# cvxopt/smcp

Measured on AMD Instinct MI355X. Metric: Newton KKT solves/sec, higher is better.
Workload: dtype f64; 1 GPU; synth50k nested block-arrow SDP n=50000, 8073 cliques, m=100; kktsolver=chol, n=50000, cliques=8073, m=100, blkval_doubles=2493568, update_doubles=10689536, parallelism=single

## Files before the change

smcp_amd/csrc/capi.hip:

```cpp
#include <hip/hip_runtime.h>
#include <memory>
#include <unordered_map>

#include <algorithm>
#include <chrono>
#include <cstdio>
#include <cstring>
#include <map>
#include <new>
#include <atomic>
#include <thread>
#include <type_traits>
#include <vector>

#include "../../include/smcp_amd.h"
#include "constraints.hpp"
#include "context.hpp"
#include "hostpar.hpp"
#include "switches.hpp"
#include "front_generic.hip"
#include "front_mfma.hip"
#include "front_large.hip"
#include "front_top.hip"
#include "front_inv.hip"
// ... 529 lines not shown
        if (dyn && tasks > c->D.ncu && tasks < ((int64_t)1 << 30) && c->D.info) {
          static bool attr2 = false;
          if (!attr2) attr2 = hipFuncSetAttribute((const void*)k_lf_assemble_lds_dyn, hipFuncAttributeMaxDynamicSharedMemorySize, 160 * 1024 - 1024) == hipSuccess;
          if (attr2) {
            int* counter = c->D.info + 24 + (st == c->aux_stream[0] ? 1 : (st == c->aux_stream[1] ? 2 : 0));
            (void)hipMemsetAsync(counter, 0, sizeof(int), st);
            launch_lds(c, KID_lf_assemble_lds_dyn, k_lf_assemble_lds_dyn, dim3(c->D.ncu), dim3(1024), bytes, st, a, U, ldu, sgn, cnt, nrhs, nz, counter);
            return;
          }
        }
        launch_lds(c, KID_lf_assemble_lds, k_lf_assemble_lds, dim3(cnt, nrhs, nz), dim3(1024), bytes, st, a, U, ldu, sgn);
        return;
      }
    }
  }
  if (a.chskip) launch(c, KID_lf_clear_upd, k_lf_zero_skipped, dim3(cnt, nrhs), dim3(256), st, a);
  if (clear_first && !(plan && a.t.gp_tptr && c->plan_full_upd))
    launch(c, KID_lf_clear_upd, k_lf_clear_upd, dim3(umax1(std::min(64, (a.namax * a.namax + 2047) / 2048)), cnt, nrhs), dim3(256), st, a);
  if (plan && a.t.gp_tptr) {
    const int nfm = a.nnmax + a.namax;
    const int gx = (int64_t)cnt * nrhs * 32 < 2 * (int64_t)c->D.ncu ? std::max(32, std::min(128, (nfm * (nfm + 1) / 2 + 255) / 256)) : 32;
    if (a.nchmax <= 8) launch(c, KID_lf_assemble, k_lf_assemble<8>, dim3(gx, cnt, nrhs), dim3(256), st, a, U, ldu, sgn);
    else launch(c, KID_lf_assemble, k_lf_assemble<16>, dim3(gx, cnt, nrhs), dim3(256), st, a, U, ldu, sgn);
    return;
  }
  const int nfmax = a.nnmax + a.namax;
  const int ncb = (nfmax + LF_TW - 1) / LF_TW, nrb = (nfmax + LF_TR - 1) / LF_TR;
  launch(c, KID_lf_assemble, k_lf_assemble_tiled, dim3(ncb * nrb, cnt, nrhs), dim3(256), st, a, U, ldu, sgn);
}

static bool pd_deep() {
  static int on = -1;
  if (on < 0) { const char* e = sw_str("SMCP_PD"); on = (e && e[0] == '1') ? 0 : 1; }
  return on == 1;
}
static int64_t pd_wgs() {
  static int64_t v = -1;
  if (v < 0) { const char* e = sw_str("SMCP_PD_WGS"); v = e ? std::max(1, atoi(e)) : 1; }
  return v;
}
#define LAUNCH_PD(c, kid, kern, grid, blk, ...)                                                        \
  do {                                                                                                 \
    const dim3 g_ = (grid);                                                                            \
    if (pd_deep() && (int64_t)g_.x * g_.y * g_.z <= pd_wgs() * (int64_t)(c)->D.ncu) launch(c, kid, kern<4>, g_, dim3(1024), __VA_ARGS__); \
    else launch(c, kid, kern<1>, g_, blk, __VA_ARGS__);                                                \
  } while (0)

constexpr int ROOT_FUSED_MAXNN = 512;
static bool root_fused() {
  static int on = -1;
  if (on < 0) { const char* e = sw_str("SMCP_ROOT_FUSED"); on = (e && e[0] == '1') ? 1 : 0; }
  return on == 1;
}
void lf_up(csp_ctx* c, const MfmaArgs& a, int cnt, int nrhs, double* U, int64_t ldu, hipStream_t st, bool fill = false) {
  const int mtA = tiles64(a.namax), ntN = tiles64(a.nnmax);
  dim3 blk(256);
  if (a.nchmax > 0) {
    lf_assemble(c, a, cnt, nrhs, U, ldu, fill ? 3 : 0, st, true);
    if (c->mid_work && a.level >= 2) {
      std::function<void(hipStream_t)> w = std::move(c->mid_work);
      c->mid_work = nullptr;
      w(st);
    }
    if (c->side_work) {
      std::function<void(hipStream_t)> w = std::move(c->side_work);
      c->side_work = nullptr;
      Fork* f = new Fork(c, st, 1);
      c->side_fork = f;
      w(f->s);
    }
  }
  LAUNCH_PD(c, KID_lf_up1, k_lf_up1, dim3(umax1(mtA * ntN + ntN * ntN), cnt, nrhs), blk, st, a, U, ldu);
  LAUNCH_PD(c, KID_lf_up2, k_lf_up2, dim3(umax1(mtA * (mtA + 1) / 2 + mtA * ntN + ntN * (ntN + 1) / 2), cnt, nrhs), blk, st, a, U, ldu);
  if (a.namax) LAUNCH_PD(c, KID_lf_up3, k_lf_up3, dim3(umax1(mtA * ntN), cnt, nrhs), blk, st, a, U, ldu);
}
void lf_down(csp_ctx* c, const MfmaArgs& a, int cnt, int nrhs, double* U, int64_t ldu, hipStream_t st) {
  const int mtA = tiles64(a.namax), ntN = tiles64(a.nnmax);
  dim3 blk(256);
  if (a.namax) launch(c, KID_gather_level, k_gather_level, dim3(cnt, nrhs, gather_parts(a.namax, (int64_t)cnt * nrhs, c->D.ncu)), dim3(NT), st, a.t, (const double*)U, ldu, a.t.upd);
  LAUNCH_PD(c, KID_lf_down1, k_lf_down1, dim3(umax1(mtA * ntN + ntN * ntN), cnt, nrhs), blk, st, a, U, ldu);
  if (a.namax) LAUNCH_PD(c, KID_lf_down2, k_lf_down2, dim3(umax1(mtA * ntN), cnt, nrhs), blk, st, a, U, ldu);
  LAUNCH_PD(c, KID_lf_down3, k_lf_down3, dim3(umax1(ntN * (ntN + 1) / 2), cnt, nrhs), blk, st, a, U, ldu);
}
void lf_pinv(csp_ctx* c, const MfmaArgs& a, int cnt, double* x, hipStream_t st) {
  const int mtA = tiles64(a.namax), ntN = tiles64(a.nnmax);
  dim3 blk(256);
  if (a.namax) {
    launch(c, KID_gather_level, k_gather_level, dim3(cnt, 1, gather_parts(a.namax, cnt, c->D.ncu)), dim3(NT), st, a.t, (const double*)x, (int64_t)0, a.t.upd);
    LAUNCH_PD(c, KID_lf_pinv1, k_lf_pinv1, dim3(umax1(mtA * ntN), cnt, 1), blk, st, a, x);
  }
  LAUNCH_PD(c, KID_lf_pinv2, k_lf_pinv2, dim3(umax1(ntN * (ntN + 1) / 2 + mtA * ntN), cnt, 1), blk, st, a, x);
}

constexpr size_t LF_DIAG_LDS = (size_t)(2 * LB * LBD + 256 + 16 * LB) * sizeof(double);
static dim3 diag_blk() {
  static int t = 0;
  if (!t) { const char* e = sw_str("SMCP_DIAG_THREADS"); t = e ? atoi(e) : 512; if (t < 64 || t > 1024 || (t & 63)) t = 512; }
  return dim3(t);
}

bool use_mid(int rowsmax) {
  static int g = -1;
  if (g < 0) {
    const char* e = sw_str("SMCP_MID");
    g = (e && e[0] == '0') ? 0 : 1;
    if (g && hipFuncSetAttribute((const void*)k_mid_chol, hipFuncAttributeMaxDynamicSharedMemorySize, (int)mid_chol_lds(MID_MAXROWS)) != hipSuccess) g = 0;
  }
  return g == 1 && rowsmax <= MID_MAXROWS;
}
bool flow_chol(csp_ctx* c, hipStream_t st, double* A, int64_t ld, int n, double* dinv, const MfmaArgs* fa, int mode, int* info, int info_val, int cnt = 1) {
  static int on = -1, wgs = 0;
  if (on < 0) { on = sw_on("SMCP_FLOW", 1); wgs = std::max(1, std::min(FLOW_MAXWG, sw_int("SMCP_FLOW_WG", FLOW_MAXWG))); }
  if (!on || use_generic(c) || n <= 2 * LB || n > FLOW_MAXN || !info) return false;
  if (cnt < 1 || (cnt > 1 && (!fa || dinv || cnt > wgs / 8))) return false;
  static int attr = -1;
  if (attr < 0) attr = hipFuncSetAttribute((const void*)k_chol_flow, hipFuncAttributeMaxDynamicSharedMemorySize, (int)FLOW_LDS_BYTES) == hipSuccess ? 1 : 0;
  if (!attr) return false;
  const int nt = (n + 63) / 64, ntiles = nt * (nt + 1) / 2;
  csp_ctx::FlowWs& W = c->flow_ws[st == c->aux_stream[0] && st ? 1 : (st == c->aux_stream[1] && st ? 2 : 0)];
  if (W.cap_nt < nt || W.cap_fronts < cnt) {
    const int ntc = std::max(nt, W.cap_nt), ntilesc = ntc * (ntc + 1) / 2, frc = std::max(cnt, W.cap_fronts);
    DevLedger& mem = c->D.mem;
    W.epoch = 0;
    if (dev_grow(&W.P, &W.len_P, (int64_t)frc * ntilesc * 4096, mem, st) || dev_grow(&W.dinv, &W.len_dinv, (int64_t)frc * ntc * 4096, mem, st) ||
        dev_grow(&W.flags, &W.len_flags, (int64_t)frc * (ntilesc + ntc + 4), mem, st) ||
        hipMemset(W.flags, 0, sizeof(unsigned) * (size_t)W.len_flags) != hipSuccess) {
      (void)hipGetLastError();
      (void)dev_free(mem, W.P, W.dinv, W.flags);
      W = csp_ctx::FlowWs();
      return false;
    }
    W.cap_nt = ntc; W.cap_fronts = frc;
  }
  const int wgs_front = cnt > 1 ? wgs / cnt : (n > 2048 ? (wgs * 10) / 7 : wgs);
  if ((int64_t)ntiles > (int64_t)FLOW_MAXOWN * wgs_front) return false;
  const int plan_key = n * 1024 + std::min(1023, wgs_front);
  auto it = c->flow_plans.find(plan_key);
  if (it == c->flow_plans.end()) {
    std::vector<int32_t> optr, otile;
    flow_make_plan(n, wgs_front, optr, otile);
    csp_ctx::FlowPlanDev P;
    P.nwg = (int)optr.size() - 1;
    if (dev_upload(&P.own_ptr, optr, c->D.mem) || dev_upload(&P.own_tile, otile, c->D.mem)) {
      (void)hipGetLastError();
      (void)dev_free(c->D.mem, P.own_ptr, P.own_tile);
      return false;
    }
    it = c->flow_plans.emplace(plan_key, P).first;
  }
  FlowArgs f;
  f.A = A; f.ld = ld; f.n = n;
  f.dinv = dinv ? dinv : W.dinv;
  f.P = W.P; f.flags = W.flags;
  f.epoch = ++W.epoch;
  f.own_ptr = it->second.own_ptr; f.own_tile = it->second.own_tile;
  f.info = info; f.info_val = info_val;
  f.cl = fa ? fa->t.cl : nullptr; f.lev = fa ? fa->t.lev : nullptr; f.mode = mode; f.nsn1 = fa ? fa->t.nsn1 : 1;
  f.dbg = nullptr;
  f.p_stride = (int64_t)ntiles * 4096; f.dinv_stride = (int64_t)nt * 4096; f.flag_stride = ntiles + nt + 4;
  static int stamps = -1;
  if (stamps < 0) stamps = sw_on("SMCP_FLOW_STAMPS", 0);
  static long long* dbg = nullptr;
  if (stamps) { if (!dbg) (void)hipMalloc((void**)&dbg, sizeof(long long) * 16 * FLOW_MAXWG); f.dbg = dbg; }
  launch_lds(c, KID_chol_flow, k_chol_flow, dim3(it->second.nwg, cnt), dim3(256), FLOW_LDS_BYTES, st, f);
  if (stamps && dbg) {
    std::vector<long long> h((size_t)8 * it->second.nwg);
    (void)hipStreamSynchronize(st);
    (void)hipMemcpy(h.data(), dbg, h.size() * sizeof(long long), hipMemcpyDeviceToHost);
    for (int w = 0; w < std::min(it->second.nwg, 20); ++w)
      fprintf(stderr, "flow n %d wg %3d: idle %7.1f us (%lld)  update %7.1f us (%lld)  potrf %7.1f us (%lld)  panel %7.1f us (%lld)\n", n, w,
              h[8 * w] / 100.0, h[8 * w + 4], h[8 * w + 1] / 100.0, h[8 * w + 5], h[8 * w + 2] / 100.0, h[8 * w + 6], h[8 * w + 3] / 100.0, h[8 * w + 7]);
// ... 1152 lines not shown
    case CSP_Q_EDM_CLAMPED:
      if (out) out[0] = c->edm_clamped;
      return 1;
    case CSP_Q_CEIG_SWEEPS:
      if (out) out[0] = c->ceig_sweeps;
      return 1;
  }
  return SMCP_EINVAL;
}

int csp_maxcardsearch(int64_t n, const int64_t* colptr, const int64_t* rowind, int64_t* order) {
  if (n <= 0 || !colptr || !rowind || !order) return SMCP_EINVAL;
  maxcardsearch(n, colptr, rowind, order);
  return 0;
}
int csp_mindegree(int64_t n, const int64_t* colptr, const int64_t* rowind, int64_t* order) {
  if (n <= 0 || !colptr || !rowind || !order) return SMCP_EINVAL;
  mindegree(n, colptr, rowind, order);
  return 0;
}
int csp_index_map(const csp_ctx* c, int64_t cnt, const int64_t* I, const int64_t* J, int64_t* out) {
  if (!c || cnt < 0) return SMCP_EINVAL;
  index_map(c->S, cnt, I, J, out);
  return 0;
}

}

#include "setup.hip"

namespace {

struct ScalFam {
  bool on = false;
  MfmaArgs af;
  int nfam = 0;
  const int32_t* lone = nullptr;
  int nlone = 0, lnn = 0, lna = 0;
  int nfmax = 0, cpan = 0, sel = 0;
  size_t bytes = 0;
};
ScalFam scaling_fam_plan(csp_ctx* c, const MfmaArgs& a0, int set) {
  ScalFam p;
  static const int on = sw_on("SMCP_SCALING_FAM", 1);
  if (!on || set || use_generic(c) || fam_off() || c->verify_cache || c->ntrial != 1 || c->sets[1].lev2 || c->sets[2].lev2 || c->S.nlev < 2) return p;
  const LevelClass& L0 = c->lvl[0];
  const LevelClass& L1 = c->lvl[1];
  if (!L1.nI || !L1.nS || !L0.nS) return p;
  for (int64_t l = 2; l < c->S.nlev; ++l) if (c->lvl[(size_t)l].nS) return p;
  if (L1.famnn > 16 || L1.famna > 64 || L1.famcnn > 16 || L1.famcna > 32) return p;
  p.af = a0;
  p.af.t.lev = c->D.lev2idx + c->S.levptr[1] + (L1.nI - L1.nS);
  p.af.level = 1;
  p.af.famna = L1.famna; p.af.famnn = L1.famnn; p.af.famcna = L1.famcna; p.af.famcnn = L1.famcnn;
  p.nfam = (int)L1.nS;
  const int nout = (int)(L0.nI - L0.nS);
  if (nout > 0 && L0.nnmaxI <= 16 && L0.namaxI <= 64) { p.lone = c->D.lev2idx + c->S.levptr[0]; p.nlone = nout; p.lnn = L0.nnmaxI; p.lna = L0.namaxI; }
  p.nfmax = std::max(L1.famnn + L1.famna, p.lnn + p.lna);
  p.cpan = (L1.famcnn + L1.famcna) * L1.famcnn;
  p.bytes = sfam_lds_bytes(p.nfmax, p.cpan);
  if (p.bytes > 64 * 1024) return p;
  const int pnat = (std::max(std::max((int)L1.famna, p.lna), 1) + 15) / 16, cnat = (std::max((int)L1.famcna, 1) + 15) / 16;
  p.sel = 2 * pnat + cnat;
  p.on = p.sel >= 3 && p.sel <= 10;
  return p;
}
template <bool PREP>
bool launch_chol_fam(csp_ctx* c, const ScalFam& p, double* x, double* lkout, hipStream_t st) {
  const dim3 grid(p.nfam + p.nlone), blk(256);
#define SMCP_CF(PN, CN) launch_lds(c, KID_chol_fam, k_chol_fam<PN, CN, PREP>, grid, blk, p.bytes, st, p.af, x, lkout, p.nfmax, p.cpan, p.nfam, p.lone); return true
  switch (p.sel) {
    case 3: SMCP_CF(1, 1);
    case 4: SMCP_CF(1, 2);
    case 5: SMCP_CF(2, 1);
    case 6: SMCP_CF(2, 2);
    case 7: SMCP_CF(3, 1);
    case 8: SMCP_CF(3, 2);
    case 9: SMCP_CF(4, 1);
    case 10: SMCP_CF(4, 2);
  }
#undef SMCP_CF
  return false;
}
bool launch_pinv_fam(csp_ctx* c, const ScalFam& p, const MfmaArgs& ap, double* x, hipStream_t st) {
  MfmaArgs af = p.af;
  af.t.upd = ap.t.upd; af.LK = ap.LK;
  const dim3 grid(p.nfam + p.nlone), blk(256);
#define SMCP_PF(PN, CN) launch_lds(c, KID_pinv_fam, k_pinv_fam<PN, CN>, grid, blk, p.bytes, st, af, x, p.nfmax, p.cpan, p.nfam, p.lone); return true
  switch (p.sel) {
    case 3: SMCP_PF(1, 1);
    case 4: SMCP_PF(1, 2);
    case 5: SMCP_PF(2, 1);
    case 6: SMCP_PF(2, 2);
    case 7: SMCP_PF(3, 1);
    case 8: SMCP_PF(3, 2);
    case 9: SMCP_PF(4, 1);
    case 10: SMCP_PF(4, 2);
  }
#undef SMCP_PF
  return false;
}
template <class Small, class Large, class Fam>
void scaling_fam_up(csp_ctx* c, const ScalFam& p, const MfmaArgs& a0, Small small, Large large, Fam fam) {
  for (int64_t l = 0; l < 2; ++l) {
    if (l == 1) fam();
    for_level_classes(c, l, a0, [&](bool lds, MfmaArgs am, int cnt, size_t, int thr) {
      if (!lds) { large(am, cnt, l); return; }
      cnt -= am.nS;
      if (cnt > 0 && !(l == 0 && p.nlone)) small(am, cnt, thr);
    });
  }
}
template <class Small, class Large, class Fam>
void scaling_fam_down(csp_ctx* c, const ScalFam& p, const MfmaArgs& a0, Small small, Large large, Fam fam) {
  for (int64_t l = 1; l >= 0; --l) {
    if (l == 0) fam();
    for_level_classes(c, l, a0, [&](bool lds, MfmaArgs am, int cnt, size_t, int thr) {
      if (!lds) { large(am, cnt, l); return; }
      cnt -= am.nS;
      if (cnt > 0 && !(l == 0 && p.nlone)) small(am, cnt, thr);
    });
  }
}

}

extern "C" {

int64_t csp_device_bytes(const csp_ctx* c) { return c ? c->D.mem.total : 0; }

static int cholesky_impl(csp_ctx* c, double* x, void* stream, int set, bool li_last = false);
int csp_cholesky(csp_ctx* c, double* x, void* stream) { return cholesky_impl(c, x, stream, 0); }
int csp_cholesky_part(csp_ctx* c, double* x, int set, void* stream) {
  if (set < 1 || set > 2 || !c || !c->sets[set].lev2 || use_generic(c)) return SMCP_EINVAL;
  return cholesky_impl(c, x, stream, set);
}
static int cholesky_impl(csp_ctx* c, double* x, void* stream, int set, bool li_last) {
  if (int rc = ready(c)) return rc;
  invalidate_tags(c, x);
  hipStream_t st = (hipStream_t)stream;
  TreeArgs a = tree_args(c);
  HIPCHK(zero_flag(c, st));
  if (!use_generic(c)) {
    MfmaArgs a0 = mfma_args(c, nullptr, 0, 1);
    a0.LK = nullptr;
    auto small = [&](const MfmaArgs& am, int cnt, int thr) {
      launch_lds(c, KID_chol_mfma, k_chol_mfma<true>, dim3(cnt), dim3(fact_threads(am, thr, 0)),
                 (size_t)mfma_lds_doubles_for(WK_CHOL, am.nnmax, am.namax) * sizeof(double), st, am, x, (double*)nullptr);
    };
    auto large = [&](const MfmaArgs& am, int cnt, int64_t l) {
      if (use_large() && c->D.gp_tptr) lf_chol(c, am, cnt, x, st, li_last && l == c->S.nlev - 1);
      else launch_lds(c, KID_chol_mfma_hbm, k_chol_mfma<false>, dim3(cnt), dim3(1024), 0, st, am, x, (double*)nullptr);
    };
    const ScalFam sf = scaling_fam_plan(c, a0, set);
    if (sf.on) scaling_fam_up(c, sf, a0, small, large, [&]() { launch_chol_fam<false>(c, sf, x, (double*)nullptr, st); });
    for (int64_t l = sf.on ? 2 : 0; l < c->S.nlev; ++l)
      for_level_classes(c, l, a0, [&](bool lds, MfmaArgs am, int cnt, size_t bytes, int thr) {
        (void)bytes;
        if (lds) small(am, cnt, thr);
        else large(am, cnt, l);
      }, set);
  } else
  for_levels_up(c, [&](const int32_t* lev, int cnt) {
    a.lev = lev;
    launch(c, KID_chol_level, k_chol_level, dim3(cnt), dim3(NT), st, a, x);
  });
  HIPCHK(end_call(c));
  return fetch_info(c, st);
}

int csp_llt(csp_ctx* c, double* x, void* stream) {
// ... 94 lines not shown
  if (c->scal_lstar < 0) {
    int64_t ls = S.nlev;
    while (ls > 0 && c->lvl[(size_t)ls - 1].nI == 0) --ls;
    c->scal_lstar = ls;
    std::vector<int> lev_of((size_t)S.nsn, 0);
    for (int64_t l = 0; l < S.nlev; ++l)
      for (int64_t q = S.levptr[l]; q < S.levptr[l + 1]; ++q) lev_of[(size_t)S.levidx[q]] = (int)l;
    int64_t t0 = bl;
    for (int64_t k = 0; k < S.nsn; ++k) if (lev_of[(size_t)k] == S.nlev - 1) t0 = std::min<int64_t>(t0, S.blkptr[k]);
    for (int64_t k = 0; k < S.nsn; ++k) if (S.blkptr[k] >= t0 && lev_of[(size_t)k] != S.nlev - 1) { t0 = 0; break; }
    c->scal_tail0 = t0;
  }
  const int64_t lstar = c->scal_lstar;
  const bool fast = !use_generic(c) && use_large() && D.gp_tptr && !cache_off() && Fork::enabled() && scaling_overlap_on() &&
                    c->ntrial == 1 && lstar < S.nlev && (lstar > 0 || D.nI_total == 0) && D.yaa && S.updlen() > 0 && !c->verify_cache;
  if (!fast) {
    const bool li = top_li_whole(c);
    if (li) { D.lk_tag_L = D.lk_tag_Y = nullptr; D.part_valid = false; D.lk_gen++; }
    if (int rc = cholesky_impl(c, L, (void*)st, 0, li)) return rc;
    HIPCHK(hipMemcpyAsync(Y, L, sizeof(double) * bl, hipMemcpyDeviceToDevice, st));
    if (int rc = projected_inverse_impl(c, Y, (void*)st, 0, li)) return rc;
    c->D.lk_tag_L = L;
    if (flags & SCALING_FAC) { if (int rc = prepare_yaa(c, Y, true, st)) return rc; HIPCHK(end_call(c)); }
    return 0;
  }
  invalidate_tags(c, L);
  invalidate_tags(c, Y);
  HIPCHK(zero_flag(c, st));
  const int64_t last = S.nlev - 1;
  const int64_t tail0 = c->scal_tail0;
  MfmaArgs a0 = mfma_args(c, nullptr, 0, 1);
  a0.LK = nullptr;
  TreeArgs t = tree_args(c);
  int nnI = 0;
  for (const LevelClass& Lc : c->lvl) if (Lc.nI) nnI = std::max(nnI, (int)Lc.nnmaxI);
  static int cprep = -1;
  if (cprep < 0) { const char* e = sw_str("SMCP_CHOL_PREP"); cprep = (e && e[0] == '0') ? 0 : 1; }
  const bool fuse_prep = cprep && nnI <= 16;
  auto chol_small = [&](const MfmaArgs& am, int cnt, int thr) {
    const size_t lb = (size_t)mfma_lds_doubles_for(WK_CHOL, am.nnmax, am.namax) * sizeof(double);
    if (fuse_prep) launch_lds(c, KID_chol_mfma, k_chol_mfma<true, true>, dim3(cnt), dim3(fact_threads(am, thr, 0)), lb, st, am, L, D.lk);
    else launch_lds(c, KID_chol_mfma, k_chol_mfma<true>, dim3(cnt), dim3(fact_threads(am, thr, 0)), lb, st, am, L, (double*)nullptr);
  };
  auto chol_large = [&](const MfmaArgs& am, int cnt, int64_t l) { lf_chol(c, am, cnt, L, st, l == last); };
  auto chol_level = [&](int64_t l) {
    for_level_classes(c, l, a0, [&](bool lds, MfmaArgs am, int cnt, size_t bytes, int thr) {
      (void)bytes;
      if (lds) chol_small(am, cnt, thr);
      else chol_large(am, cnt, l);
    });
  };
  const ScalFam sf = scaling_fam_plan(c, a0, 0);
  if (sf.on)
    scaling_fam_up(c, sf, a0, chol_small, chol_large, [&]() {
      if (fuse_prep) launch_chol_fam<true>(c, sf, L, D.lk, st);
      else launch_chol_fam<false>(c, sf, L, (double*)nullptr, st);
    });
  for (int64_t l = sf.on ? 2 : 0; l < last; ++l) chol_level(l);
  std::unique_ptr<Fork> f0;
  if (last > 0) f0.reset(new Fork(c, st, 1));
  hipStream_t s0 = f0 ? f0->s : st;
  chol_level(last);
  if (D.nI_total && !fuse_prep) {
    TreeArgs ts = t;
    ts.lev = D.lev3idx;
    launch_lds(c, KID_prep_lk, k_prep_lk, dim3((int)D.nI_total), dim3(prep_lk_threads(nnI)), prep_lk_lds_bytes(nnI), s0, ts, (const double*)L, D.lk);
  }
  for (int64_t ll = 0; ll < last; ++ll)
    for_level_classes(c, ll, a0, [&](bool lds, MfmaArgs am, int cnt, size_t, int) { if (!lds) lf_prep(c, am, cnt, L, s0); });
  if (tail0 > 0) (void)hipMemcpyAsync(Y, L, sizeof(double) * tail0, hipMemcpyDeviceToDevice, s0);
  for_level_classes(c, last, a0, [&](bool lds, MfmaArgs am, int cnt, size_t, int) { if (!lds) lf_prep(c, am, cnt, L, st, use_top(am.nnmax + am.namax)); });
  (void)hipMemcpyAsync(Y + tail0, L + tail0, sizeof(double) * (bl - tail0), hipMemcpyDeviceToDevice, st);
  if (f0) f0->join();
  D.lk_gen++;
  D.part_valid = false;
  MfmaArgs ap = mfma_args(c, nullptr, 0, 1);
  ap.t.upd = D.yaa;
  MfmaArgs af = mfma_args(c, nullptr, 0, 1);
  const bool want_fac = (flags & SCALING_FAC) != 0;
  static int skipenv = -1;
  if (skipenv < 0) { const char* e = sw_str("SMCP_FAC_PARTIAL"); skipenv = (e && e[0] == '0') ? 0 : 1; }
  const bool skip_children = want_fac && skipenv && D.m > 0 && !D.ns && leafgram_ok(c, D.m) && c->leafgram_policy != 0;
  bool skipped = false;
  auto factor_level = [&](int64_t l, hipStream_t lds_stream, hipStream_t large_stream) {
    for_level_classes(c, l, af, [&](bool lds, MfmaArgs am, int cnt, size_t, int) {
      if (!am.namax) return;
      if (lds) {
        if (l == 0 && skip_children && am.nS > 0) { cnt -= am.nS; skipped = true; if (!cnt) return; }
        const size_t bytes = ((size_t)padld(am.namax) * am.namax + 256 + 8) * sizeof(double);
        launch_lds(c, KID_factor_yaa_lds, k_factor_yaa_lds, dim3(cnt), dim3(fact_threads(am, 256, 2)), bytes, lds_stream, am, (const double*)D.yaa, D.fac);
      } else {
        launch(c, KID_axpby, k_copy_upd_blocks, dim3(cnt, umax1(std::min(64, (am.namax * am.namax + 1023) / 1024))), dim3(256), large_stream,
               am.t, (const double*)D.yaa, D.fac);
        lf_factor_yaa(c, am, cnt, D.fac, large_stream);
      }
    });
  };
  auto pinv_small = [&](const MfmaArgs& am, int cnt, int thr) {
    launch_lds(c, KID_pinv_mfma, k_pinv_mfma<true>, dim3(cnt), dim3(fact_threads(am, thr, 1)),
               (size_t)mfma_lds_doubles_for(WK_PINV, am.nnmax, am.namax) * sizeof(double), st, am, Y);
  };
  auto pinv_large = [&](const MfmaArgs& am, int cnt, int64_t) { lf_pinv(c, am, cnt, Y, st); };
  auto pinv_level = [&](int64_t l) {
    for_level_classes(c, l, ap, [&](bool lds, MfmaArgs am, int cnt, size_t bytes, int thr) {
      (void)bytes;
      if (lds) pinv_small(am, cnt, thr);
      else pinv_large(am, cnt, l);
    });
  };
  for (int64_t l = last; l >= lstar; --l) pinv_level(l);
  bool any_large_sep = false;
  for (int64_t l = lstar; l <= last; ++l) if (c->lvl[(size_t)l].nII && c->lvl[(size_t)l].namaxII > 0) any_large_sep = true;
  std::unique_ptr<Fork> f1;
  if (want_fac && any_large_sep && lstar > 0) f1.reset(new Fork(c, st, 0));
  hipStream_t s1 = f1 ? f1->s : st;
  for (int64_t l = lstar - 1; l >= (sf.on ? 2 : 0); --l) pinv_level(l);
  if (sf.on) scaling_fam_down(c, sf, ap, pinv_small, pinv_large, [&]() { launch_pinv_fam(c, sf, ap, Y, st); });
  if (want_fac) {
    for (int64_t l = last; l >= lstar; --l) factor_level(l, s1, s1);
    for (int64_t l = lstar - 1; l >= 0; --l) factor_level(l, st, st);
  }
  if (f1) f1->join();
  D.lk_tag_L = L; D.lk_tag_Y = Y;
  D.yaa_tag = Y;
  D.fac_tag = want_fac ? Y : nullptr;
  D.fac_partial = want_fac && skipped;
  D.faci_tag = nullptr;
  if (want_fac) D.fac_gen++;
  HIPCHK(end_call(c));
  const int rc = fetch_info(c, st);
  if (rc) {
    D.lk_tag_L = D.lk_tag_Y = D.yaa_tag = D.fac_tag = D.faci_tag = nullptr;
    D.part_valid = false;
  }
  return rc;
}
int csp_cholesky_projected_inverse(csp_ctx* c, double* L, double* Y, int with_factors, void* stream) {
  if (int rc = ready(c)) return rc;
  if (!L || !Y || L == Y) return SMCP_EINVAL;
  return scaling_impl(c, L, Y, with_factors ? SCALING_FAC : 0, (hipStream_t)stream);
}

int csp_completion(csp_ctx* c, double* x, void* stream) {
  if (int rc = ready(c)) return rc;
  invalidate_tags(c, x);
  hipStream_t st = (hipStream_t)stream;
  TreeArgs a = tree_args(c);
  HIPCHK(zero_flag(c, st));
  if (!use_generic(c)) {
    prepare_yaa(c, x, true, st, true);
    MfmaArgs a0 = mfma_args(c, c->D.faci, 0, 1);
    a0.LK = nullptr;
    dim3 blk(256);
    for (int64_t l = 0; l < c->S.nlev; ++l)
      for_level_classes(c, l, a0, [&](bool lds, MfmaArgs am, int cnt, size_t bytes, int thr) {
        const size_t cb = lds ? (size_t)completion_lds_doubles(am.nnmax, am.namax) * sizeof(double) : 0;
        if (lds && cb <= LDS_LIMIT) {
          launch_lds(c, KID_completion_mfma, k_completion_mfma<true>, dim3(cnt), dim3(cb > 48 * 1024 ? 512 : 256), cb, st, am, x);
        }
        else if (lds || !use_large())
          launch_lds(c, KID_completion_mfma_hbm, k_completion_mfma<false>, dim3(cnt), dim3(lds ? 256 : thr), 0, st, am, x);
      });
    if (use_large())
      for_all_large(c, a0, [&](MfmaArgs am, int cnt) {
        const int mtA = tiles64(am.namax), ntN = tiles64(am.nnmax);
        if (am.namax) {
          launch(c, KID_lf_completion, k_lf_completion, dim3(umax1(mtA * ntN), cnt), blk, st, am, x, 0);
          launch(c, KID_lf_completion, k_lf_completion, dim3(umax1(mtA * ntN), cnt), blk, st, am, x, 1);
        }
        launch(c, KID_lf_completion, k_lf_completion, dim3(umax1(ntN * ntN), cnt), blk, st, am, x, 2);
        if (use_mid(am.nnmax))
          launch_lds(c, KID_mid_chol, k_mid_chol, dim3(cnt), dim3(1024), mid_chol_lds(am.nnmax), st, am, (double*)nullptr, (double*)nullptr, 3);
        else
        for (int jb = 0; jb < am.nnmax; jb += LB) {
          launch_lds(c, KID_lf_diag, k_lf_diag, dim3(cnt), diag_blk(), LF_DIAG_LDS, st, am, (double*)nullptr, (double*)nullptr, 3, jb, 1);
          const int mrem = am.nnmax - jb - 1;
          if (mrem > 0) {
            launch(c, KID_lf_chol_panel, k_lf_chol_panel, dim3(umax1(tiles64(mrem)), cnt), blk, st, am, (double*)nullptr, (double*)nullptr, 3, jb);
            const int mt = tiles64(mrem);
            launch(c, KID_lf_chol_trail, k_lf_chol_trail, dim3(umax1(mt * (mt + 1) / 2), cnt), blk, st, am, (double*)nullptr, (double*)nullptr, 3, jb);
          }
        }
        for (int ib = 0; ib < am.nnmax; ib += LB) {
          launch_lds(c, KID_lf_diag, k_lf_diag, dim3(cnt), diag_blk(), LF_DIAG_LDS, st, am, (double*)nullptr, (double*)nullptr, 3, ib, 0);
          if (ib > 0) launch(c, KID_lf_prep_s, k_lf_prep_s, dim3(umax1(tiles64(ib)), cnt), blk, st, am, (const double*)nullptr, (double*)nullptr, ib, 3);
          launch(c, KID_lf_prep_row, k_lf_prep_row, dim3(umax1(tiles64(ib) + 1), cnt), blk, st, am, (const double*)nullptr, (double*)nullptr, ib, 3, 0);
        }
        launch(c, KID_lf_completion, k_lf_completion, dim3(umax1(ntN * ntN + mtA * ntN), cnt), blk, st, am, x, 3);
      });
    invalidate_tags(c, x);
  } else {
    gather_all(c, x, 0, 1, c->D.upd, st);
    launch(c, KID_completion_all, k_completion_all, dim3((int)c->S.nsn), dim3(NT), st, a, x);
  }
  HIPCHK(end_call(c));
  return fetch_info(c, st);
}

int csp_hessian(csp_ctx* c, const double* L, const double* Y, double* U, int64_t nrhs, int64_t ldu,
                int adj, int inv, void* stream) {
  if (int rc = ready(c)) return rc;
  if (nrhs < 1 || adj < 0 || adj > 2 || (nrhs > 1 && ldu < c->S.blklen())) return SMCP_EINVAL;
// ... 286 lines not shown
```

smcp_amd/csrc/front_pinvfam.hip:

```cpp
#include <hip/hip_runtime.h>

namespace smcp {

template <int NAT, bool OWN, int M>
__device__ inline d4 pinv_fam_tiles(const double (&li)[4], const double (&kk)[4 * M], const CliqueDesc& d, double* P, double* yaa,
                                    double* zs, int nfz, const int32_t* rel, int t0, int t1, bool with_li, int lane) {
  const int l15 = lane & 15, kq = lane >> 4;
  const int nn = d.nn, na = d.na, nf = nn + na;
  const int ksn = (nn + 3) >> 2, ksa = (na + 3) >> 2;
  const d4 zero4 = {0.0, 0.0, 0.0, 0.0};
  d4 accN = zero4;
  if (with_li) {
#pragma unroll
    for (int s = 0; s < 4; ++s)
      if (s < ksn) fmma(accN, li[s], li[s]);
  }
#pragma unroll
  for (int t = 0; t < NAT; ++t) {
    if (t < t0 || t >= t1 || 16 * t >= na) continue;
    const int m = 16 * t + l15;
    int ri = 0;
    if (!OWN) ri = rel[min(m, na - 1)];
    d4 accE = zero4;
#pragma unroll
    for (int s0 = 0; s0 < 4 * NAT; s0 += 8) {
      double y[8];
#pragma unroll
      for (int s = s0; s < s0 + 8 && s < 4 * NAT; ++s) {
        const int j = kq + 4 * s;
        const int i1 = OWN ? nn + min(m, na - 1) : ri, j1 = OWN ? nn + min(j, na - 1) : rel[min(j, na - 1)];
        const double v = zs[pk_low(max(i1, j1), min(i1, j1), nfz)];
        y[s - s0] = (m < na && j < na) ? v : 0.0;
        if (!OWN && m < na && j <= m) yaa[m + j * na] = v;
      }
#pragma unroll
      for (int s = s0; s < s0 + 8 && s < 4 * NAT; ++s)
        if (s < ksa) fmma(accE, kk[s], y[s - s0]);
    }
#pragma unroll
    for (int rr = 0; rr < 4; ++rr) {
      const int mm = 16 * t + kq + 4 * rr;
      if (mm < na && l15 < nn) {
        P[nn + mm + l15 * nf] = -accE[rr];
        if (OWN) zs[pk_low(nn + mm, l15, nfz)] = -accE[rr];
      }
    }
#pragma unroll
    for (int s = 0; s < 4; ++s) fmma(accN, kk[4 * t + s], accE[s]);
  }
  return accN;
}

template <int PNAT, int CNAT>
__global__ void __launch_bounds__(256, 4) k_pinv_fam(MfmaArgs a, double* x, int nfmax, int cpan, int nfam, const int32_t* lone) {
  extern __shared__ double zs[];
  const int tid = threadIdx.x;
  const int lane = tid & 63, l15 = lane & 15, kq = lane >> 4;
  const int wave = __builtin_amdgcn_readfirstlane((int)(threadIdx.x >> 6));
  const int k = (int)blockIdx.x < nfam ? a.t.lev[blockIdx.x] : lone[(int)blockIdx.x - nfam];
  const CliqueDesc d = a.t.cl[k];
  const int nn = d.nn, na = d.na, nf = nn + na;
  const int nch = (int)blockIdx.x < nfam ? d.chend - d.chbeg : 0;
  double* const P = x + d.blk;
  const bool has0 = wave < nch, has1 = wave + 4 < nch;
  const CliqueDesc dc0 = a.t.cl[has0 ? a.t.chidx[d.chbeg + wave] : k];
  const CliqueDesc dc1 = a.t.cl[has1 ? a.t.chidx[d.chbeg + wave + 4] : k];
  const SfamStage st = sfam_stage_of(zs, nfmax, wave, cpan);
  if (has0) { sfam_stage(st, a.LK + dc0.blk, (dc0.nn + dc0.na) * dc0.nn, lane); sfam_stage_rel(st, a.t, dc0, lane); }
  constexpr int M = PNAT > CNAT ? PNAT : CNAT;
  double li[4], kk[4 * M];
  down_fam_load_lk<PNAT, M>(li, kk, a.LK + d.blk, d, lane);
  if (na > 0) {
    const bool haspar = d.parent >= 0;
    const CliqueDesc par = a.t.cl[haspar ? d.parent : k];
    const int nng = par.nn, nag = par.na, nfg = nng + nag;
    const double* Pg = x + par.blk;
    const double* Ug = a.t.upd + par.upd;
    double* const UkG = a.t.upd + d.upd;
    const int32_t* rel = a.t.relidx + d.rel;
    const int gi = rel[min(lane, na - 1)];
    double v[4 * PNAT];
#pragma unroll
    for (int c = 0; c < 4 * PNAT; ++c) {
      const int j = wave + 4 * c;
      v[c] = 0.0;
      if (haspar && j < na && lane >= j && lane < na) {
        const int gj = rel[j];
        const int hi = max(gi, gj), lo = min(gi, gj);
        v[c] = lo < nng ? Pg[hi + (int64_t)lo * nfg] : Ug[(hi - nng) + (int64_t)(lo - nng) * nag];
      }
    }
#pragma unroll
    for (int c = 0; c < 4 * PNAT; ++c) {
      const int j = wave + 4 * c;
      if (j < na && lane >= j && lane < na) {
        zs[pk_low(nn + lane, nn + j, nf)] = v[c];
        if (haspar) UkG[lane + j * na] = v[c];
      }
    }
  }
  __syncthreads();
  {
    const d4 accN = pinv_fam_tiles<PNAT, true, M>(li, kk, d, P, nullptr, zs, nf, nullptr, wave, wave + 1, wave == 0, lane);
#pragma unroll
    for (int rr = 0; rr < 4; ++rr) st.D[l15 + 16 * (kq + 4 * rr)] = accN[rr];
  }
  __syncthreads();
  {
    const int i = tid & 15, j = tid >> 4;
    if (i < nn && j <= i) {
      double v = sfam_stage_of(zs, nfmax, 0, cpan).D[tid];
#pragma unroll
      for (int w = 1; w < 4; ++w)
        if (w < PNAT && 16 * w < na) v += sfam_stage_of(zs, nfmax, w, cpan).D[tid];
      zs[pk_low(i, j, nf)] = v;
      P[i + j * nf] = v;
    }
  }
  if (nch == 0) return;
  __syncthreads();
  const int pan1 = (dc1.nn + dc1.na) * dc1.nn;
  const bool pre1 = has1 && pan1 <= 256;
  SfamPre pre;
  if (has0) {
    down_fam_load_lk<CNAT, M>(li, kk, st.P, dc0, lane);
    if (pre1) sfam_fetch(pre, a.LK + dc1.blk, pan1, a.t, dc1, lane);
  }
  auto child = [&](const CliqueDesc& dc) {
    double* const Pc = x + dc.blk;
    const d4 accN = pinv_fam_tiles<CNAT, false, M>(li, kk, dc, Pc, a.t.upd + dc.upd, zs, nf, st.rel, 0, CNAT, true, lane);
    const int nfc = dc.nn + dc.na;
#pragma unroll
    for (int rr = 0; rr < 4; ++rr) {
      const int c = kq + 4 * rr;
      if (l15 < dc.nn && c <= l15) Pc[l15 + c * nfc] = accN[rr];
    }
  };
  if (has0) child(dc0);
  if (has1) {
    wave_sync();
    if (pre1) sfam_commit(st, pre, pan1, dc1, lane);
    else { sfam_stage(st, a.LK + dc1.blk, pan1, lane); sfam_stage_rel(st, a.t, dc1, lane); }
    wave_sync();
    down_fam_load_lk<CNAT, M>(li, kk, st.P, dc1, lane);
    child(dc1);
  }
}

}
```

smcp_amd/csrc/switches.hpp:

```cpp
#pragma once
#include <cstdio>
#include <cstdlib>
#include <cstring>
#include <string>

extern char** environ;

namespace smcp {

struct Switch { const char* name; const char* dflt; const char* doc; };

static const Switch SWITCHES[] = {
  {"SMCP_GENERIC", "0", "1: any-size fixed-order kernels of front_generic.hip for every tree operation (as CSP_TUNE_DETERMINISTIC)"},
  {"SMCP_LARGE", "1", "0: no tiled large-front kernels (fronts beyond LDS take the one-workgroup HBM kernels)"},
  {"SMCP_NOCACHE", "0", "1: nothing derived from (L, Y) is reused between calls"},
  {"SMCP_FORK", "1", "0: no side streams, everything on the caller's stream"},
  {"SMCP_AUX_PRIO", "1", "0: side stream 0 (few-workgroup chains) at default instead of highest priority"},
  {"SMCP_AUX_PRIO1", "1", "0: side stream 1 (filler work) at default instead of lowest priority"},
  {"SMCP_EVENT_SYSFENCE", "0", "1: internal events with the default system-scope release (12 us per hand-over instead of 7)"},
  {"SMCP_SCALING_OVERLAP", "1", "0: csp_cholesky_projected_inverse as its three steps one after the other"},
  {"SMCP_CHOL_PREP", "1", "0: k_prep_lk in a launch of its own instead of inside k_chol_mfma (narrow supernodes)"},
  {"SMCP_FAC_PARTIAL", "1", "0: chol(Y_AA) of the family children always formed by the fused scaling point"},
  {"SMCP_MID", "1", "0: per-step kernels instead of k_mid_chol / k_lf_diag_inv for fronts of at most 272 rows"},
  {"SMCP_TOP_FUSED", "1", "0: k_mid_chol, and k_lf_diag_inv / k_lf_trtri for the inverse at the scaling point, instead of the register-resident k_top_chol for fronts of at most 208 rows"},
  {"SMCP_TRTRI", "1", "0: block-row triangular inversion of large fronts instead of recursive doubling"},
  {"SMCP_N16", "1", "0: no shape-specialised k_hess_up_n16"},
  {"SMCP_OLDLDS", "0", "1: k_hess_up_mfma<true> instead of the padded / n16 kernels"},
  {"SMCP_DOWN_W", "1", "0: k_hess_down_mfma instead of the one-wave k_hess_down_w"},
  {"SMCP_DOWN_FAM", "1", "most right-hand sides of a root -> leaves sweep that take the one-launch family kernel k_hess_down_fam (0: never; the per-level k_hess_down_w launches)"},
  {"SMCP_UP_FAM", "1", "most dense right-hand sides of a leaves -> root sweep that take the resident family kernel k_hess_up_fam1, the level-0 cliques outside the families riding along (0: never; k_hess_up_fam and a launch of their own for those cliques)"},
  {"SMCP_SCALING_FAM", "1", "0: per-level k_chol_mfma / k_pinv_mfma launches for the families of the scaling point instead of one k_chol_fam / k_pinv_fam launch each way"},
  {"SMCP_FAM", "1", "0: no family kernels (per-level sweeps with the update exchange through HBM)"},
  {"SMCP_FAM2", "1", "0: no sparse-input family kernels (k_fam_sparse, k_fam_terms): k_hess_up_fam"},
  {"SMCP_FAMT", "1", "0: no entry-driven family sweep k_fam_terms (k_fam_sparse instead)"},
  {"SMCP_FZ", "1", "0: the family parents' packed updates go through HBM (k_fam_terms writes, the extend-add reads) instead of being formed by k_lf_assemble_fz"},
  {"SMCP_FAMT_GROUP", "1", "0: no sibling groups of family parents (k_fam_terms_grp)"},
  {"SMCP_LFSP", "1", "0: dense phases instead of the sparse-input sweep k_lfsp_up of childless large fronts"},
  {"SMCP_LFSP_GROUP", "1", "0: no sibling groups in k_lfsp_up"},
  {"SMCP_ZSP", "1", "0: dense first phase of wide childless fronts instead of k_lf_zsp"},
  {"SMCP_LEAFGRAM", "1", "0: never the closed-form Gram blocks of the family children (k_leaf_tables / k_leaf_pairs)"},
  {"SMCP_LG_SIDE", "1", "0: leaf Gram blocks after the sweep on the caller's stream instead of beside the top phases"},
  {"SMCP_GRAM_EARLY", "0", "1: the Gram chunks of the levels 0 / 1 rows on the side branch beside the top fronts' phase kernels (measured slower: 3.37 against 3.22 ms per step)"},
  {"SMCP_LG_EARLY", "1", "0: leaf Gram blocks beside the phase kernels of the top fronts instead of from the start of the sweep"},
  {"SMCP_FACI_LDS", "1", "0: inverse Y_AA factors of the small fronts by block rows against HBM (k_factor_inverse) instead of in LDS"},
  {"SMCP_FZ_TAIL", "1", "0: every (front, right-hand side) pair of the fused extend-add is one workgroup's task, also in a thin last round"},
  {"SMCP_GRAM", "1", "0: reference (two-sweep) formulation of the Schur complement instead of the Gram formulation"},
  {"SMCP_SCM", "1", "0: column-sparse constraints swept like the others (no SCMcolumn2 route)"},
  {"SMCP_TRSM_MM", "1", "0: csp_trsm through the generic level kernels instead of tile products"},
  {"SMCP_TRMM_MM", "1", "0: no MFMA tile products in csp_trmm (every front on the FMA kernels); 2: tile products for the large fronts only, also from 32 columns on"},
  {"SMCP_SYR2K_MM", "1", "0: no MFMA tile products in csp_syr2k (every front on the FMA kernel); 2: tile products for the large fronts only, whatever the rank (read on every call)"},
  {"SMCP_SYMM_MM", "1", "0: no MFMA tile products in csp_symm (every front on the FMA kernel); 2: tile products for the large fronts only, whatever the column count (read on every call)"},
  {"SMCP_LOWRANK_MM", "1", "0: no MFMA tiles in the Gram products of the low-rank factor (k_lr_gram on the FMA route whatever the shape)"},
  {"SMCP_POTRS_MANY_MM", "1", "0: no MFMA tile products in the block steps of dense_potrs_many / kkt_solve_many (FMA updates whatever the column count; read on every call)"},
  {"SMCP_ALDS", "1", "0: extend-add of large fronts by gather plan only (no LDS streaming kernel)"},
  {"SMCP_ALDS_DYN", "1", "0: one workgroup per (front, right-hand side) instead of the task-drawing grid"},
  {"SMCP_ALDS_FILL", "1", "0: k_panel_fill builds the input panels instead of the extend-add (sgn 3)"},
  {"SMCP_ASM", "plan", "t: tiled extend-add kernel instead of the gather plan"},
  {"SMCP_ROOT_FUSED", "0", "1: fused two-product sweep of fronts without separator (Y_NN explicit: condition squared; studies only)"},
  {"SMCP_PD", "0", "1: four-wave tile products everywhere (no sixteen-wave shape for small launches)"},
  {"SMCP_FLOW", "1", "0: no one-launch blocked Cholesky with in-launch tile dataflow (front_flow.hip): per-step kernels for dense matrices / single fronts beyond 272 rows"},
  {"SMCP_FLOW_WG", "112", "workgroups of that launch (at most 112: four launches fit the chip side by side)"},
  {"SMCP_POTRF_DEFER", "1", "0: kkt_schur_factor factors H at once even under deferred status"},
  {"SMCP_QR_TRSM", "mfma", "f: vector-FMA substitution kernel of kkt_qr instead of the MFMA one"},
  {"SMCP_FTHR_CHOL", "128", "threads of k_chol_mfma on the leaf class"},
  {"SMCP_FTHR_PINV", "256", "threads of k_pinv_mfma on the leaf class"},
  {"SMCP_FTHR_YAA", "64", "threads of k_factor_yaa_lds on the leaf class"},
  {"SMCP_FTHR_YAA_MID", "256", "threads of k_factor_yaa_lds on separator blocks of 33 .. 64 rows"},
  {"SMCP_N16_THR_LEAF", "128", "threads of k_hess_up_n16 for one or two right-hand sides on childless fronts"},
  {"SMCP_DIAG_THREADS", "512", "threads of k_lf_diag"},
  {"SMCP_POTRF_THREADS", "1024", "threads of k_dense_potrf_small"},
  {"SMCP_FZ_THREADS", "1024", "threads of k_lf_assemble_fz (512: eight waves, no register spills, slower)"},
  {"SMCP_PD_WGS", "1", "largest launch, in workgroups per CU, that takes the sixteen-wave tile shape"},
  {"SMCP_ALDS_Z", "0", "workgroups per (front, right-hand side) of the LDS extend-add (0: automatic)"},
  {"SMCP_RHS_SPLIT", "16", "fewest right-hand sides for the two-stream split of a large-front sweep (plain extend-add launch only)"},
  {"SMCP_RHS_PARTS", "2", "parts of that split (2 or 3)"},
  {"SMCP_RHS_SPLIT_DYN", "0", "1: the split also with the task-drawing extend-add"},
  {"SMCP_FAM_MINRHS", "1", "fewest dense right-hand sides for the family kernel"},
  {"SMCP_FAMT_G", "0", "right-hand-side slices per family of k_fam_terms (0: cost model)"},
  {"SMCP_FAM2_STAG", "0", "stagger of k_fam_sparse's groups (studies)"},
  {"SMCP_FAMT_MEAN", "36", "entry-driven family sweeps (k_fam_terms, fused extend-add) up to this many entries per (family, constraint) list ON AVERAGE (lists up to 384 entries, in chunks); beyond: the dense family sweep"},
  {"SMCP_LFSP_OCC", "2", "waves per SIMD the grouped update phase of k_lfsp_up is compiled for (1: 512 registers, no spills; 2: 256, ~100 spilled)"},
  {"SMCP_LFSP_G", "1", "right-hand sides per workgroup of k_lfsp_up"},
  {"SMCP_GRAM_NW", "16", "waves per workgroup of k_gram_diag128 (4, 8 or 16)"},
  {"SMCP_GRAM_MINCHUNK", "512", "fewest stack rows per workgroup of the Gram accumulation"},
  {"SMCP_UPDP_PAD", "0", "doubles of padding between the packed exchange buffers of consecutive right-hand sides"},
  {"SMCP_QR_PASSES", "0", "Cholesky-QR passes of kkt_qr (0: decided by the deviation test)"},
  {"SMCP_QR_P", "1", "positions per lane of the FMA substitution kernel (1 or 2)"},
  {"SMCP_FLOW_STAMPS", "0", "1: per-workgroup time accounts of the one-launch blocked Cholesky on stderr (waits for every launch)"},
  {"SMCP_POISON", "0", "1: every fp64 device buffer of the library (and the exchange buffers of smcp_amd/kkt.py) starts as 4.5e150 (hunting reads of never-written workspace)"},
  {"SMCP_RACE", "0", "seed > 0: delay injection on every internal stream hand-over and one launch in eight (race hunting; results must not change)"},
  {"SMCP_TRACE", "0", "1: every launch named on stderr and waited for (a device fault points at its kernel)"},
  {"SMCP_TIMING", "0", "1: wall-clock marks of the set-up phases on stderr"},
  {"SMCP_OCC", "0", "1: occupancy decisions of k_hess_up_n16 on stderr"},
  {"SMCP_DEBUG_ADDR", "0", "1: addresses of the large allocations on stderr"},
  {"SMCP_CONTIG", "0", "1: large buffers from physically contiguous memory (placement studies: slower)"},
  {"SMCP_SKIP", "0", "phase mask of the sweep kernels (ablation timing; results are wrong)"},
  {"SMCP_GSKIP", "0", "ablation mask of the Gram kernel (results are wrong)"},
  {"SMCP_LGSKIP", "0", "ablation mask of k_leaf_pairs (results are wrong)"},
  {"SMCP_QR_FAKE", "0", "1: timing experiment of the FMA substitution kernel (results are wrong)"},
};

inline void sw_check_environment() {
  static const bool done = [] {
    for (char** e = environ; e && *e; ++e) {
      if (std::strncmp(*e, "SMCP_", 5) != 0) continue;
      const char* eq = std::strchr(*e, '=');
      const std::string name(*e, eq ? (size_t)(eq - *e) : std::strlen(*e));
      if (name.rfind("SMCP_BENCH_", 0) == 0 || name.rfind("SMCP_FUZZ_", 0) == 0 || name == "SMCP_CXXFLAGS" || name == "SMCP_STAMPS" ||
          name == "SMCP_SHARD_KEEP" || name == "SMCP_SHARD_TOP" || name == "SMCP_GIT_SHA" || name == "SMCP_FS_MODE") continue;
      bool known = false;
      for (const Switch& s : SWITCHES) if (name == s.name) known = true;
      if (!known) std::fprintf(stderr, "smcp_amd: unknown switch %s in the environment (see smcp_amd/csrc/switches.hpp)\n", name.c_str());
    }
    return true;
// ... 15 lines not shown
```

Measured before the change: 356.2 KKT solves/s.

## Fuse Y_AA factorization of family parents into k_pinv_fam and start side factoring early

At the scaling point, the Cholesky/inverse of Y_AA for family parents and lone level-0 cliques is now computed inside k_pinv_fam from the LDS-resident Y front. The separate k_factor_yaa_lds launches for those cliques are skipped, which saves launches and HBM re-reads. The large-front factor levels are also queued on the side stream right after the gather at level lstar, so they overlap the rest of the pinv sweep. In exchange the family kernel needs more LDS, which can lower occupancy, and the stream ordering becomes more complex.

Result: no change. 358.8 KKT solves/s, median of 6 (+0.7%).

```diff
diff --git a/smcp_amd/csrc/capi.hip b/smcp_amd/csrc/capi.hip
--- a/smcp_amd/csrc/capi.hip
+++ b/smcp_amd/csrc/capi.hip
@@ -635,11 +635,12 @@
   if (a.namax) LAUNCH_PD(c, KID_lf_down2, k_lf_down2, dim3(umax1(mtA * ntN), cnt, nrhs), blk, st, a, U, ldu);
   LAUNCH_PD(c, KID_lf_down3, k_lf_down3, dim3(umax1(ntN * (ntN + 1) / 2), cnt, nrhs), blk, st, a, U, ldu);
 }
-void lf_pinv(csp_ctx* c, const MfmaArgs& a, int cnt, double* x, hipStream_t st) {
+void lf_pinv(csp_ctx* c, const MfmaArgs& a, int cnt, double* x, hipStream_t st, const std::function<void()>* gathered = nullptr) {
   const int mtA = tiles64(a.namax), ntN = tiles64(a.nnmax);
   dim3 blk(256);
   if (a.namax) {
     launch(c, KID_gather_level, k_gather_level, dim3(cnt, 1, gather_parts(a.namax, cnt, c->D.ncu)), dim3(NT), st, a.t, (const double*)x, (int64_t)0, a.t.upd);
+    if (gathered) (*gathered)();
     LAUNCH_PD(c, KID_lf_pinv1, k_lf_pinv1, dim3(umax1(mtA * ntN), cnt, 1), blk, st, a, x);
   }
   LAUNCH_PD(c, KID_lf_pinv2, k_lf_pinv2, dim3(umax1(ntN * (ntN + 1) / 2 + mtA * ntN), cnt, 1), blk, st, a, x);
@@ -1958,11 +1959,16 @@
 #undef SMCP_CF
   return false;
 }
-bool launch_pinv_fam(csp_ctx* c, const ScalFam& p, const MfmaArgs& ap, double* x, hipStream_t st) {
+bool launch_pinv_fam(csp_ctx* c, const ScalFam& p, const MfmaArgs& ap, double* x, hipStream_t st, double* fac = nullptr, int nfac = 0) {
   MfmaArgs af = p.af;
   af.t.upd = ap.t.upd; af.LK = ap.LK;
   const dim3 grid(p.nfam + p.nlone), blk(256);
-#define SMCP_PF(PN, CN) launch_lds(c, KID_pinv_fam, k_pinv_fam<PN, CN>, grid, blk, p.bytes, st, af, x, p.nfmax, p.cpan, p.nfam, p.lone); return true
+  const int fna = std::max((int)p.af.famna, p.lna);
+  const size_t bytes = fac ? std::max(p.bytes, ((size_t)padld(fna) * fna + 256 + 8) * sizeof(double)) : p.bytes;
+#define SMCP_PF(PN, CN) \
+  if (fac) launch_lds(c, KID_pinv_fam, k_pinv_fam<PN, CN, true>, grid, blk, bytes, st, af, x, p.nfmax, p.cpan, p.nfam, p.lone, fac, nfac); \
+  else launch_lds(c, KID_pinv_fam, k_pinv_fam<PN, CN, false>, grid, blk, bytes, st, af, x, p.nfmax, p.cpan, p.nfam, p.lone, (double*)nullptr, 0); \
+  return true
   switch (p.sel) {
     case 3: SMCP_PF(1, 1);
     case 4: SMCP_PF(1, 2);
@@ -2223,11 +2229,17 @@
   if (skipenv < 0) { const char* e = sw_str("SMCP_FAC_PARTIAL"); skipenv = (e && e[0] == '0') ? 0 : 1; }
   const bool skip_children = want_fac && skipenv && D.m > 0 && !D.ns && leafgram_ok(c, D.m) && c->leafgram_policy != 0;
   bool skipped = false;
+  static const int famfac = sw_on("SMCP_PINV_FAM_FAC", 1);
+  const bool fam_fac = sf.on && want_fac && famfac;
+  const bool fam_fac_lone = fam_fac && sf.nlone > 0 && skip_children;
   auto factor_level = [&](int64_t l, hipStream_t lds_stream, hipStream_t large_stream) {
     for_level_classes(c, l, af, [&](bool lds, MfmaArgs am, int cnt, size_t, int) {
       if (!am.namax) return;
       if (lds) {
-        if (l == 0 && skip_children && am.nS > 0) { cnt -= am.nS; skipped = true; if (!cnt) return; }
+        if (l == 0 && skip_children && am.nS > 0) { cnt -= am.nS; skipped = true; }
+        if (l == 0 && fam_fac_lone) cnt -= sf.nlone;
+        if (l == 1 && fam_fac) cnt -= am.nS;
+        if (cnt <= 0) return;
         const size_t bytes = ((size_t)padld(am.namax) * am.namax + 256 + 8) * sizeof(double);
         launch_lds(c, KID_factor_yaa_lds, k_factor_yaa_lds, dim3(cnt), dim3(fact_threads(am, 256, 2)), bytes, lds_stream, am, (const double*)D.yaa, D.fac);
       } else {
@@ -2241,7 +2253,16 @@
     launch_lds(c, KID_pinv_mfma, k_pinv_mfma<true>, dim3(cnt), dim3(fact_threads(am, thr, 1)),
                (size_t)mfma_lds_doubles_for(WK_PINV, am.nnmax, am.namax) * sizeof(double), st, am, Y);
   };
-  auto pinv_large = [&](const MfmaArgs& am, int cnt, int64_t) { lf_pinv(c, am, cnt, Y, st); };
+  bool any_large_sep = false;
+  for (int64_t l = lstar; l <= last; ++l) if (c->lvl[(size_t)l].nII && c->lvl[(size_t)l].namaxII > 0) any_large_sep = true;
+  std::unique_ptr<Fork> f1;
+  const bool early_side = fam_fac && any_large_sep && lstar > 0;
+  const std::function<void()> hand_over = [&]() {
+    if (f1) return;
+    f1.reset(new Fork(c, st, 0));
+    for (int64_t l = last; l >= lstar; --l) factor_level(l, f1->s, f1->s);
+  };
+  auto pinv_large = [&](const MfmaArgs& am, int cnt, int64_t l) { lf_pinv(c, am, cnt, Y, st, (early_side && l == lstar) ? &hand_over : nullptr); };
   auto pinv_level = [&](int64_t l) {
     for_level_classes(c, l, ap, [&](bool lds, MfmaArgs am, int cnt, size_t bytes, int thr) {
       (void)bytes;
@@ -2250,15 +2271,17 @@
     });
   };
   for (int64_t l = last; l >= lstar; --l) pinv_level(l);
-  bool any_large_sep = false;
-  for (int64_t l = lstar; l <= last; ++l) if (c->lvl[(size_t)l].nII && c->lvl[(size_t)l].namaxII > 0) any_large_sep = true;
-  std::unique_ptr<Fork> f1;
-  if (want_fac && any_large_sep && lstar > 0) f1.reset(new Fork(c, st, 0));
+  const bool side_queued = (bool)f1;
+  if (!f1 && want_fac && any_large_sep && lstar > 0) f1.reset(new Fork(c, st, 0));
   hipStream_t s1 = f1 ? f1->s : st;
   for (int64_t l = lstar - 1; l >= (sf.on ? 2 : 0); --l) pinv_level(l);
-  if (sf.on) scaling_fam_down(c, sf, ap, pinv_small, pinv_large, [&]() { launch_pinv_fam(c, sf, ap, Y, st); });
+  if (sf.on)
+    scaling_fam_down(c, sf, ap, pinv_small, pinv_large, [&]() {
+      if (fam_fac) launch_pinv_fam(c, sf, ap, Y, st, D.fac, sf.nfam + (fam_fac_lone ? sf.nlone : 0));
+      else launch_pinv_fam(c, sf, ap, Y, st);
+    });
   if (want_fac) {
-    for (int64_t l = last; l >= lstar; --l) factor_level(l, s1, s1);
+    if (!side_queued) for (int64_t l = last; l >= lstar; --l) factor_level(l, s1, s1);
     for (int64_t l = lstar - 1; l >= 0; --l) factor_level(l, st, st);
   }
   if (f1) f1->join();
diff --git a/smcp_amd/csrc/front_pinvfam.hip b/smcp_amd/csrc/front_pinvfam.hip
--- a/smcp_amd/csrc/front_pinvfam.hip
+++ b/smcp_amd/csrc/front_pinvfam.hip
@@ -51,8 +51,59 @@
   return accN;
 }
 
-template <int PNAT, int CNAT>
-__global__ void __launch_bounds__(256, 4) k_pinv_fam(MfmaArgs a, double* x, int nfmax, int cpan, int nfam, const int32_t* lone) {
+template <int PNAT>
+__device__ inline void pinv_fam_factor(double* zs, const TreeArgs& t, int k, const CliqueDesc& d, double* fac, int wave, int lane) {
+  const int nn = d.nn, na = d.na, nf = nn + na;
+  const int ld = padld(na);
+  double* const M = zs;
+  double* const D16 = zs + ld * na;
+  int* const verdict = (int*)(D16 + 256);
+  double v[4 * PNAT];
+  __syncthreads();
+#pragma unroll
+  for (int c = 0; c < 4 * PNAT; ++c) {
+    const int j = wave + 4 * c;
+    v[c] = (j < na && lane >= j && lane < na) ? zs[pk_low(nn + lane, nn + j, nf)] : 0.0;
+  }
+  __syncthreads();
+#pragma unroll
+  for (int c = 0; c < 4 * PNAT; ++c) {
+    const int j = wave + 4 * c;
+    if (j < na && lane < na) M[lane + j * ld] = v[c];
+  }
+  for (int jb = 0; jb < na; jb += 16) {
+    const int bw = min(16, na - jb);
+    __syncthreads();
+    if (wave == 0) {
+      const bool ok = wave_potrf_inv16(M + jb + jb * ld, ld, bw, D16);
+      if (lane == 0) *verdict = ok ? 0 : 1;
+    }
+    __syncthreads();
+    if (*verdict) { if (threadIdx.x == 0) atomicCAS(info_of(t, k), 0, info_val(t, k)); return; }
+    const int mrem = na - jb - bw;
+    if (mrem > 0) {
+      double* Pj = M + (jb + bw) + jb * ld;
+      wg_mma(mrem, bw, bw, [=](int m, int kk) { return Pj[m + kk * ld]; },
+             [=](int kk, int n) { return D16[n + kk * 16]; },
+             [=](int m, int n, double acc) { Pj[m + n * ld] = acc; });
+      __syncthreads();
+      double* Tr = M + (jb + bw) + (jb + bw) * ld;
+      wg_mma(mrem, mrem, bw, [=](int m, int kk) { return Pj[m + kk * ld]; },
+             [=](int kk, int n) { return Pj[n + kk * ld]; },
+             [=](int m, int n, double acc) { if (m >= n) Tr[m + n * ld] -= acc; }, true);
+    }
+  }
+  __syncthreads();
+  double* const dst = fac + d.upd;
+#pragma unroll
+  for (int c = 0; c < 4 * PNAT; ++c) {
+    const int j = wave + 4 * c;
+    if (j < na && lane >= j && lane < na) dst[lane + j * na] = M[lane + j * ld];
+  }
+}
+
+template <int PNAT, int CNAT, bool FAC>
+__global__ void __launch_bounds__(256, 4) k_pinv_fam(MfmaArgs a, double* x, int nfmax, int cpan, int nfam, const int32_t* lone, double* fac, int nfac) {
   extern __shared__ double zs[];
   const int tid = threadIdx.x;
   const int lane = tid & 63, l15 = lane & 15, kq = lane >> 4;
@@ -117,7 +168,8 @@
       P[i + j * nf] = v;
     }
   }
-  if (nch == 0) return;
+  if (!FAC && nch == 0) return;
+  if (!FAC || nch > 0) {
   __syncthreads();
   const int pan1 = (dc1.nn + dc1.na) * dc1.nn;
   const bool pre1 = has1 && pan1 <= 256;
@@ -145,6 +197,10 @@
     down_fam_load_lk<CNAT, M>(li, kk, st.P, dc1, lane);
     child(dc1);
   }
-}
-
-}
+  }
+  if constexpr (FAC) {
+    if ((int)blockIdx.x < nfac && na > 0) pinv_fam_factor<PNAT>(zs, a.t, k, d, fac, wave, lane);
+  }
+}
+
+}
diff --git a/smcp_amd/csrc/switches.hpp b/smcp_amd/csrc/switches.hpp
--- a/smcp_amd/csrc/switches.hpp
+++ b/smcp_amd/csrc/switches.hpp
@@ -30,6 +30,7 @@
   {"SMCP_DOWN_FAM", "1", "most right-hand sides of a root -> leaves sweep that take the one-launch family kernel k_hess_down_fam (0: never; the per-level k_hess_down_w launches)"},
   {"SMCP_UP_FAM", "1", "most dense right-hand sides of a leaves -> root sweep that take the resident family kernel k_hess_up_fam1, the level-0 cliques outside the families riding along (0: never; k_hess_up_fam and a launch of their own for those cliques)"},
   {"SMCP_SCALING_FAM", "1", "0: per-level k_chol_mfma / k_pinv_mfma launches for the families of the scaling point instead of one k_chol_fam / k_pinv_fam launch each way"},
+  {"SMCP_PINV_FAM_FAC", "1", "0: chol(Y_AA) of the family parents and of the lone cliques riding along by k_factor_yaa_lds launches behind k_pinv_fam instead of inside it (the fused scaling point with factors)"},
   {"SMCP_FAM", "1", "0: no family kernels (per-level sweeps with the update exchange through HBM)"},
   {"SMCP_FAM2", "1", "0: no sparse-input family kernels (k_fam_sparse, k_fam_terms): k_hess_up_fam"},
   {"SMCP_FAMT", "1", "0: no entry-driven family sweep k_fam_terms (k_fam_sparse instead)"},
```
